# EdoardoBotta/RQ-VAE-Recommender

Hardware: AMD Instinct MI355X
Metric: item-embeddings quantized/sec (RQ-VAE fwd+bwd) (higher is better)
Workload: dtype f32 (MLP GEMMs f16x2-emulated)

## Files before the change

rq-vae-recommender_amd/csrc/wgrad_split.hip:

```cpp
#include "rqhip_common.h"

namespace rqhip {

typedef float ws_f32x16 __attribute__((ext_vector_type(16)));
typedef float ws_f32x4 __attribute__((ext_vector_type(4)));
typedef float ws_f32x2 __attribute__((ext_vector_type(2)));
typedef __bf16 ws_bf16x8 __attribute__((ext_vector_type(8)));
typedef __bf16 ws_bf16x2 __attribute__((ext_vector_type(2)));
typedef unsigned ws_u32x2 __attribute__((ext_vector_type(2)));

constexpr int kWsRows = 16;

#ifndef WS_PROBE
#define WS_PROBE 0
#endif

struct WgradSplitParams {
    const float *g, *y, *x;
    float *gm, *out;
    long long M;
    int N, K;
    int nslab_n, nslab_k, msplit;
    long long n_chunks;
    const unsigned *g_max, *x_max;
};

__device__ __forceinline__ void ws_split2(float a, float b, unsigned &h, unsigned &m, unsigned &l) {
    const ws_bf16x2 hh = __builtin_convertvector(ws_f32x2{a, b}, ws_bf16x2);
    h = __builtin_bit_cast(unsigned, hh);
    const float ra = a - __builtin_bit_cast(float, h << 16), rb = b - __builtin_bit_cast(float, h & 0xffff0000u);
    const ws_bf16x2 mm = __builtin_convertvector(ws_f32x2{ra, rb}, ws_bf16x2);
    m = __builtin_bit_cast(unsigned, mm);
    const float sa = ra - __builtin_bit_cast(float, m << 16), sb = rb - __builtin_bit_cast(float, m & 0xffff0000u);
    const ws_bf16x2 ll = __builtin_convertvector(ws_f32x2{sa, sb}, ws_bf16x2);
    l = __builtin_bit_cast(unsigned, ll);
}

typedef _Float16 ws_f16x8 __attribute__((ext_vector_type(8)));
typedef _Float16 ws_f16x2 __attribute__((ext_vector_type(2)));
__device__ __forceinline__ void ws_split2_f16(float a, float b, unsigned &h, unsigned &m) {
    const ws_f16x2 hh = __builtin_convertvector(ws_f32x2{a, b}, ws_f16x2);
    h = __builtin_bit_cast(unsigned, hh);
    const ws_f32x2 hf = __builtin_convertvector(hh, ws_f32x2);
    const ws_f16x2 mm = __builtin_convertvector(ws_f32x2{a - hf.x, b - hf.y}, ws_f16x2);
    m = __builtin_bit_cast(unsigned, mm);
}
__device__ __forceinline__ int ws_exp_of_bits(unsigned b) {
    b &= 0x7fffffffu;
    const int e = (int)(b >> 23);
    return (b == 0u || e == 255) ? 0 : (e == 0 ? -126 : e - 127) - 14;
}

__device__ __forceinline__ ws_f32x4 ws_load4(const float *p) {
    ws_f32x4 v;
    asm volatile("global_load_dwordx4 %0, %1, off" : "=v"(v) : "v"(p));
    return v;
}
template <int N>
__device__ __forceinline__ void ws_await(ws_f32x4 (&r)[4]) {
    asm volatile("s_waitcnt vmcnt(%4)" : "+v"(r[0]), "+v"(r[1]), "+v"(r[2]), "+v"(r[3]) : "n"(N) : "memory");
}

template <int TA, int TB, int WA, int WB, bool MASK, int NP>
__device__ __forceinline__ void wgrad_split_body(const WgradSplitParams &p, const int block) {
    constexpr int Nt = 32 * TA * WA, Kt = 32 * TB * WB, NT = 64 * WA * WB;
    constexpr int UNITS = Nt + Kt;
    constexpr int UQ = (UNITS + NT - 1) / NT;
    constexpr int SG = Nt / 4 + 4, SX = Kt / 4 + 4;
    constexpr int PART_G = NP * 2 * 4 * SG * 4, PART_X = NP * 2 * 4 * SX * 4;
    extern __shared__ __attribute__((aligned(16))) char ws_smem[];
    unsigned *sbuf = reinterpret_cast<unsigned *>(ws_smem);

    const int tid = threadIdx.x, lane = tid & 63, wave = tid >> 6;
    const int il = lane & 31, h = lane >> 5;
    const int wa = wave / WB, wb = wave % WB;
    const int nslabs = p.nslab_n * p.nslab_k;
    int slab, split;
    if ((p.msplit & 7) == 0) {
        const int xcd = block & 7, j = block >> 3;
        slab = j % nslabs;
        split = (j / nslabs) * 8 + xcd;
    } else {
        slab = block % nslabs;
        split = block / nslabs;
    }
    const int slab_n = slab / p.nslab_k, slab_k = slab % p.nslab_k;
    const int n0 = slab_n * Nt, k0 = slab_k * Kt;
    const long long r_begin = (p.n_chunks * split / p.msplit) * 32;
    long long r_end = (p.n_chunks * (split + 1) / p.msplit) * 32;
    if (r_end > p.M) r_end = p.M;
    const long long n_stage = (r_end - r_begin + kWsRows - 1) / kWsRows;
    const bool write_back = MASK && p.gm != nullptr && slab_k == 0;

    ws_f32x16 acc[TA][TB];
#pragma unroll
    for (int t = 0; t < TA; ++t)
#pragma unroll
        for (int u = 0; u < TB; ++u)
#pragma unroll
            for (int r = 0; r < 16; ++r) acc[t][u][r] = 0.0f;

    ws_f32x4 rv0[UQ][4], rv1[UQ][4], ry[MASK ? UQ : 1][4];
    int ue[NP == 2 ? UQ : 1][4];
#pragma unroll
    for (int q = 0; q < (NP == 2 ? UQ : 0); ++q) {
        const int u = tid + q * NT;
        const bool isg = u < Nt;
        const int idx = isg ? u : u - Nt, W = isg ? Nt : Kt;
        const int cq = idx % (W / 4);
        const unsigned *mxp = isg ? p.g_max : p.x_max;
        const int c0 = isg ? n0 : k0;
#pragma unroll
        for (int cc = 0; cc < 4; ++cc)
            ue[q][cc] = (mxp && ((UNITS % NT == 0) || u < UNITS)) ? ws_exp_of_bits(mxp[c0 + 4 * cq + cc]) : 0;
    }
    const long long n_full = (r_end - r_begin) / kWsRows;
    const float *cur[UQ][4];
    const float *ycur[MASK ? UQ : 1][4];
    size_t step16[UQ];
#pragma unroll
    for (int q = 0; q < UQ; ++q) {
        const int u = tid + q * NT;
        const bool live = (UNITS % NT == 0) || u < UNITS;
        const bool isg = u < Nt;
        const int idx = live ? (isg ? u : u - Nt) : 0, W = isg ? Nt : Kt;
        const int cq = idx % (W / 4), rq = idx / (W / 4);
        const int ld = isg ? p.N : p.K, c0 = isg ? n0 : k0;
        step16[q] = (size_t)kWsRows * ld;
#pragma unroll
        for (int j = 0; j < 4; ++j) {
            const size_t off = (size_t)(r_begin + 4 * rq + j) * ld + c0 + 4 * cq;
            cur[q][j] = (isg ? p.g : p.x) + off;
            if (MASK) ycur[q][j] = p.y + (isg ? off : (size_t)0);
        }
    }
    auto fetch_tail = [&](long long stage, ws_f32x4 (&rv)[UQ][4]) {
        const long long row0 = r_begin + stage * kWsRows;
#pragma unroll
        for (int q = 0; q < UQ; ++q) {
            const int u = tid + q * NT;
            const bool live = (UNITS % NT == 0) || u < UNITS;
            const bool isg = u < Nt;
            const int idx = live ? (isg ? u : u - Nt) : 0, W = isg ? Nt : Kt;
            const int cq = idx % (W / 4), rq = idx / (W / 4);
            const float *base = isg ? p.g : p.x;
            const int ld = isg ? p.N : p.K, c0 = isg ? n0 : k0;
#pragma unroll
            for (int j = 0; j < 4; ++j) {
                const long long row = row0 + 4 * rq + j;
                const bool ok = live && row < r_end;
                const size_t off = (size_t)(ok ? row : 0) * ld + c0 + 4 * cq;
                rv[q][j] = ok ? *reinterpret_cast<const ws_f32x4 *>(base + off) : ws_f32x4{0.f, 0.f, 0.f, 0.f};
                if (MASK) ry[q][j] = (ok && isg) ? *reinterpret_cast<const ws_f32x4 *>(p.y + off) : ws_f32x4{1.f, 1.f, 1.f, 1.f};
            }
        }
    };
    auto fetch = [&](long long stage, ws_f32x4 (&rv)[UQ][4]) {
        if (stage >= n_full) {
            fetch_tail(stage, rv);
            return;
        }
#pragma unroll
        for (int q = 0; q < UQ; ++q) {
            const int u = tid + q * NT;
            const bool live = (UNITS % NT == 0) || u < UNITS;
            const bool isg = u < Nt;
#pragma unroll
            for (int j = 0; j < 4; ++j) {
                if constexpr ((WS_PROBE & 2) != 0) {
                    rv[q][j] = ws_f32x4{1.f + (float)stage, 2.f, 3.f, 4.f};
                    if (MASK) ry[q][j] = ws_f32x4{1.f, 1.f, 1.f, 1.f};
                } else {
                    const ws_f32x4 v = *reinterpret_cast<const ws_f32x4 *>(cur[q][j]);
                    rv[q][j] = live ? v : ws_f32x4{0.f, 0.f, 0.f, 0.f};
                    if (MASK) {
                        const ws_f32x4 yv = *reinterpret_cast<const ws_f32x4 *>(ycur[q][j]);
                        ry[q][j] = (live && isg) ? yv : ws_f32x4{1.f, 1.f, 1.f, 1.f};
                    }
                }
                cur[q][j] += step16[q];
                if (MASK && isg) ycur[q][j] += step16[q];
            }
        }
    };
    auto stash = [&](long long stage, int buf, ws_f32x4 (&rv)[UQ][4]) {
        const long long row0 = r_begin + stage * kWsRows;
        unsigned *dst = sbuf + buf * (PART_G + PART_X);
        if (WS_PROBE & 1) return;
#pragma unroll
        for (int q = 0; q < UQ; ++q) {
            const int u = tid + q * NT;
            if (UNITS % NT != 0 && u >= UNITS) continue;
            const bool isg = u < Nt;
            const int idx = isg ? u : u - Nt, W = isg ? Nt : Kt;
            const int cq = idx % (W / 4), rq = idx / (W / 4);
            if (MASK && isg) {
#pragma unroll
                for (int j = 0; j < 4; ++j) {
                    rv[q][j].x = ry[q][j].x <= 0.0f ? 0.0f : rv[q][j].x;
                    rv[q][j].y = ry[q][j].y <= 0.0f ? 0.0f : rv[q][j].y;
                    rv[q][j].z = ry[q][j].z <= 0.0f ? 0.0f : rv[q][j].z;
                    rv[q][j].w = ry[q][j].w <= 0.0f ? 0.0f : rv[q][j].w;
                }
                if (write_back) {
#pragma unroll
                    for (int j = 0; j < 4; ++j) {
                        const long long row = row0 + 4 * rq + j;
                        if (row < r_end) *reinterpret_cast<ws_f32x4 *>(p.gm + (size_t)row * p.N + n0 + 4 * cq) = rv[q][j];
                    }
                }
            }
            unsigned *part = dst + (isg ? 0 : PART_G);
            const int oct = rq >> 1, half = rq & 1, S4 = 4 * (isg ? SG : SX);
#pragma unroll
            for (int cc = 0; cc < 4; ++cc) {
                unsigned h01, m01, l01 = 0u, h23, m23, l23 = 0u;
                if constexpr (NP == 2) {
                    ws_split2_f16(ldexpf(rv[q][0][cc], -ue[q][cc]), ldexpf(rv[q][1][cc], -ue[q][cc]), h01, m01);
                    ws_split2_f16(ldexpf(rv[q][2][cc], -ue[q][cc]), ldexpf(rv[q][3][cc], -ue[q][cc]), h23, m23);
                } else {
                    ws_split2(rv[q][0][cc], rv[q][1][cc], h01, m01, l01);
                    ws_split2(rv[q][2][cc], rv[q][3][cc], h23, m23, l23);
                }
                const int pos = cc * (S4 / 4) + cq;
                *reinterpret_cast<ws_u32x2 *>(part + ((0 * 2 + oct) * S4 + pos) * 4 + 2 * half) = ws_u32x2{h01, h23};
                *reinterpret_cast<ws_u32x2 *>(part + ((1 * 2 + oct) * S4 + pos) * 4 + 2 * half) = ws_u32x2{m01, m23};
                if (NP == 3) *reinterpret_cast<ws_u32x2 *>(part + ((2 * 2 + oct) * S4 + pos) * 4 + 2 * half) = ws_u32x2{l01, l23};
            }
        }
    };

    const bool stage_first = wave < (WA * WB) / 2;
    auto multiply = [&](int buf) {
        const ws_bf16x8 *gA = reinterpret_cast<const ws_bf16x8 *>(sbuf + buf * (PART_G + PART_X));
        const ws_bf16x8 *xB = reinterpret_cast<const ws_bf16x8 *>(sbuf + buf * (PART_G + PART_X) + PART_G);
        ws_bf16x8 a[TA][NP], b[TB][NP];
#pragma unroll
        for (int t = 0; t < TA; ++t)
#pragma unroll
            for (int pc = 0; pc < NP; ++pc)
                a[t][pc] = (WS_PROBE & 8) ? ws_bf16x8{(__bf16)(float)(t + buf), 1, 2, 3, 4, 5, 6, 7}
                                          : gA[(pc * 2 + h) * (4 * SG) + (il & 3) * SG + ((wa * 32 * TA + 32 * t + il) >> 2)];
#pragma unroll
        for (int u = 0; u < TB; ++u)
#pragma unroll
            for (int pc = 0; pc < NP; ++pc)
                b[u][pc] = (WS_PROBE & 8) ? ws_bf16x8{(__bf16)(float)(u + buf), 1, 2, 3, 4, 5, 6, 7}
                                          : xB[(pc * 2 + h) * (4 * SX) + (il & 3) * SX + ((wb * 32 * TB + 32 * u + il) >> 2)];
#pragma unroll
        for (int t = 0; t < TA; ++t)
#pragma unroll
            for (int u = 0; u < TB; ++u) {
                ws_f32x16 c16 = acc[t][u];
                if constexpr ((WS_PROBE & 4) != 0) {
                    c16[0] += (float)a[t][0][0] + (float)b[u][0][1] + (float)a[t][NP - 1][2] + (float)b[u][NP - 1][3];
                } else if constexpr (NP == 2) {
                    c16 = __builtin_amdgcn_mfma_f32_32x32x16_f16(__builtin_bit_cast(ws_f16x8, a[t][1]), __builtin_bit_cast(ws_f16x8, b[u][0]), c16, 0, 0, 0);
                    c16 = __builtin_amdgcn_mfma_f32_32x32x16_f16(__builtin_bit_cast(ws_f16x8, a[t][0]), __builtin_bit_cast(ws_f16x8, b[u][1]), c16, 0, 0, 0);
                    c16 = __builtin_amdgcn_mfma_f32_32x32x16_f16(__builtin_bit_cast(ws_f16x8, a[t][0]), __builtin_bit_cast(ws_f16x8, b[u][0]), c16, 0, 0, 0);
                } else {
                    c16 = __builtin_amdgcn_mfma_f32_32x32x16_bf16(a[t][1], b[u][1], c16, 0, 0, 0);
                    c16 = __builtin_amdgcn_mfma_f32_32x32x16_bf16(a[t][NP - 1], b[u][0], c16, 0, 0, 0);
                    c16 = __builtin_amdgcn_mfma_f32_32x32x16_bf16(a[t][0], b[u][NP - 1], c16, 0, 0, 0);
                    c16 = __builtin_amdgcn_mfma_f32_32x32x16_bf16(a[t][1], b[u][0], c16, 0, 0, 0);
                    c16 = __builtin_amdgcn_mfma_f32_32x32x16_bf16(a[t][0], b[u][1], c16, 0, 0, 0);
                    c16 = __builtin_amdgcn_mfma_f32_32x32x16_bf16(a[t][0], b[u][0], c16, 0, 0, 0);
                }
                acc[t][u] = c16;
            }
    };
    constexpr bool kTwoSets = !MASK && UQ == 1 && WS_PROBE == 0;
    if constexpr (!kTwoSets) {
        if (n_stage > 0) {
            fetch(0, rv0);
            stash(0, 0, rv0);
            if (n_stage > 1) fetch(1, rv0);
        }
        __syncthreads();
        for (long long c = 0; c < n_stage; ++c) {
            const int buf = (int)(c & 1);
            if (stage_first) {
                if (c + 1 < n_stage) stash(c + 1, buf ^ 1, rv0);
                if (c + 2 < n_stage) fetch(c + 2, rv0);
            }
            multiply(buf);
            if (!stage_first) {
                if (c + 1 < n_stage) stash(c + 1, buf ^ 1, rv0);
                if (c + 2 < n_stage) fetch(c + 2, rv0);
            }
            if (!(WS_PROBE & 16)) __syncthreads();
        }
    } else {
        auto load_set = [&](ws_f32x4 (&r)[UQ][4]) {
#pragma unroll
            for (int j = 0; j < 4; ++j) {
                r[0][j] = ws_load4(cur[0][j]);
                cur[0][j] += step16[0];
            }
        };
        long long c = 0;
        if (n_full >= 5) {
            load_set(rv0);
            load_set(rv1);
            ws_await<4>(rv0[0]);
            stash(0, 0, rv0);
            load_set(rv0);
            __syncthreads();
            if (stage_first) {
                for (; c + 4 < n_full; c += 2) {
                    ws_await<4>(rv1[0]);
                    stash(c + 1, 1, rv1);
                    load_set(rv1);
                    multiply(0);
                    __syncthreads();
                    ws_await<4>(rv0[0]);
                    stash(c + 2, 0, rv0);
                    load_set(rv0);
                    multiply(1);
                    __syncthreads();
                }
                ws_await<0>(rv1[0]);
                ws_await<0>(rv0[0]);
            } else {
                for (; c + 4 < n_full; c += 2) {
                    multiply(0);
                    ws_await<4>(rv1[0]);
                    stash(c + 1, 1, rv1);
                    load_set(rv1);
                    __syncthreads();
                    multiply(1);
                    ws_await<4>(rv0[0]);
                    stash(c + 2, 0, rv0);
                    load_set(rv0);
                    __syncthreads();
                }
                ws_await<0>(rv1[0]);
                ws_await<0>(rv0[0]);
            }
        } else {
            if (n_stage > 0) fetch(0, rv0);
            if (n_stage > 1) fetch(1, rv1);
            if (n_stage > 0) stash(0, 0, rv0);
            if (n_stage > 2) fetch(2, rv0);
            __syncthreads();
        }
        for (; c < n_stage; c += 2) {
            if (stage_first) {
                if (c + 1 < n_stage) stash(c + 1, 1, rv1);
                if (c + 3 < n_stage) fetch(c + 3, rv1);
            }
            multiply(0);
            if (!stage_first) {
                if (c + 1 < n_stage) stash(c + 1, 1, rv1);
                if (c + 3 < n_stage) fetch(c + 3, rv1);
            }
            __syncthreads();
            if (c + 1 >= n_stage) break;
            if (stage_first) {
                if (c + 2 < n_stage) stash(c + 2, 0, rv0);
                if (c + 4 < n_stage) fetch(c + 4, rv0);
            }
            multiply(1);
            if (!stage_first) {
                if (c + 2 < n_stage) stash(c + 2, 0, rv0);
                if (c + 4 < n_stage) fetch(c + 4, rv0);
            }
            __syncthreads();
        }
    }

    float *dst = p.out + (size_t)split * p.N * p.K;
    int ek[TB];
#pragma unroll
    for (int u = 0; u < TB; ++u) ek[u] = (NP == 2 && p.x_max) ? ws_exp_of_bits(p.x_max[k0 + wb * 32 * TB + 32 * u + il]) : 0;
    typedef unsigned ws_u32x4 __attribute__((ext_vector_type(4)));
    ws_u32x4 gb[TA][4];
#pragma unroll
    for (int t = 0; t < TA; ++t)
#pragma unroll
        for (int g4 = 0; g4 < 4; ++g4)
            gb[t][g4] = (NP == 2 && p.g_max) ? *reinterpret_cast<const ws_u32x4 *>(p.g_max + n0 + wa * 32 * TA + 32 * t + 8 * g4 + 4 * h)
                                             : ws_u32x4{0u, 0u, 0u, 0u};
#pragma unroll
    for (int t = 0; t < TA; ++t) {
#pragma unroll
        for (int u = 0; u < TB; ++u)
#pragma unroll
            for (int r = 0; r < 16; ++r) {
                const int n = n0 + wa * 32 * TA + 32 * t + 8 * (r >> 2) + 4 * h + (r & 3);
                const int k = k0 + wb * 32 * TB + 32 * u + il;
                float v = acc[t][u][r];
                if constexpr (NP == 2) v = ldexpf(v, ws_exp_of_bits(gb[t][r >> 2][r & 3]) + ek[u]);
                dst[(size_t)n * p.K + k] = v;
            }
    }
}

template <int TA, int TB, int WA, int WB, bool MASK, int NP>
__global__ __launch_bounds__(64 * WA * WB) void wgrad_split_kernel(const WgradSplitParams p) {
    wgrad_split_body<TA, TB, WA, WB, MASK, NP>(p, (int)blockIdx.x);
}

constexpr int kWsMaxJobs = 4;
struct WgradSplitJobs {
    WgradSplitParams p[kWsMaxJobs];
    int first[kWsMaxJobs];
    int n;
};
template <int TA, int TB, int WA, int WB, int NP>
__global__ __launch_bounds__(64 * WA * WB) void wgrad_split_jobs_kernel(const WgradSplitJobs jobs) {
    WgradSplitParams p = jobs.p[0];
    int first = 0;
#pragma unroll
    for (int j = 1; j < kWsMaxJobs; ++j)
        if (j < jobs.n && (int)blockIdx.x >= jobs.first[j]) {
            p = jobs.p[j];
            first = jobs.first[j];
        }
    wgrad_split_body<TA, TB, WA, WB, false, NP>(p, (int)blockIdx.x - first);
}

struct WgradSplitJobsMixed {
    WgradSplitJobs jobs;
    int cfg[kWsMaxJobs];
};
template <int NP>
__global__ __launch_bounds__(512) void wgrad_split_jobs_mixed_kernel(const WgradSplitJobsMixed m) {
    WgradSplitParams p = m.jobs.p[0];
    int first = 0, cfg = m.cfg[0];
#pragma unroll
    for (int j = 1; j < kWsMaxJobs; ++j)
        if (j < m.jobs.n && (int)blockIdx.x >= m.jobs.first[j]) {
            p = m.jobs.p[j];
            first = m.jobs.first[j];
            cfg = m.cfg[j];
        }
    if (cfg == 1) wgrad_split_body<2, 2, 2, 4, false, NP>(p, (int)blockIdx.x - first);
    else wgrad_split_body<2, 2, 4, 2, false, NP>(p, (int)blockIdx.x - first);
}

int wgrad_split_cfg(int N, int K) {
    if (N % 256 == 0 && K % 256 == 0) return 0;
    if (N % 128 == 0 && K % 256 == 0) return 1;
    if (N % 256 == 0 && K % 128 == 0) return 2;
    return -1;
}

template <int TA, int TB, int WA, int WB, int NP>
static int wgrad_split_go(const WgradSplitParams &p, bool mask, hipStream_t s) {
    constexpr int Nt = 32 * TA * WA, Kt = 32 * TB * WB;
    const size_t lds = (size_t)2 * (4 * (Nt / 4 + 4) + 4 * (Kt / 4 + 4)) * NP * 2 * 16;
    auto go = [&](auto kern) -> int {
        static LdsGrant grant;
        RQ_RETURN_IF_HIP(grant.ensure(reinterpret_cast<const void *>(kern), 160 * 1024));
        hipLaunchKernelGGL(kern, dim3(p.nslab_n * p.nslab_k * p.msplit), dim3(64 * WA * WB), lds, s, p);
        RQ_CHECK_LAUNCH("wgrad_split_kernel");
        return 0;
    };
    return mask ? go(wgrad_split_kernel<TA, TB, WA, WB, true, NP>) : go(wgrad_split_kernel<TA, TB, WA, WB, false, NP>);
}

int launch_wgrad_split(int cfg, const float *g, const float *y, const float *x, long long M, int N, int K, float *gm, float *out,
                       int nslab_n, int nslab_k, int msplit, const unsigned *g_max, const unsigned *x_max, hipStream_t s) {
    WgradSplitParams p;
    p.g = g; p.y = y; p.x = x; p.gm = gm; p.out = out;
    p.M = M; p.N = N; p.K = K; p.nslab_n = nslab_n; p.nslab_k = nslab_k; p.msplit = msplit;
    p.n_chunks = (M + 31) / 32;
    p.g_max = g_max;
    p.x_max = x_max;
    const bool mask = y != nullptr;
    if (g_max && x_max) {
        switch (cfg) {
            case 0: return wgrad_split_go<4, 2, 2, 4, 2>(p, mask, s);
            case 1: return wgrad_split_go<2, 2, 2, 4, 2>(p, mask, s);
            default: return wgrad_split_go<2, 2, 4, 2, 2>(p, mask, s);
        }
    }
    switch (cfg) {
        case 0: return wgrad_split_go<4, 2, 2, 4, 3>(p, mask, s);
        case 1: return wgrad_split_go<2, 2, 2, 4, 3>(p, mask, s);
        default: return wgrad_split_go<2, 2, 4, 2, 3>(p, mask, s);
    }
}

int launch_wgrad_split_jobs(int n, const float *const *g, const float *const *x, long long M, const int *N, const int *K, float *const *out,
                            int msplit, const unsigned *const *g_max, const unsigned *const *x_max, int half, hipStream_t s) {
    WgradSplitJobsMixed m;
    WgradSplitJobs &jobs = m.jobs;
    jobs.n = n;
    int blocks = 0;
    for (int j = 0; j < kWsMaxJobs; ++j) {
        const int i = j < n ? j : 0;
        const int cfg = half ? wgrad_split_cfg(N[i], K[i]) : 0;
        const int Nt = cfg == 1 ? 128 : 256, Kt = cfg == 2 ? 128 : 256;
        WgradSplitParams &p = jobs.p[j];
        p.g = g[i]; p.y = nullptr; p.x = x[i]; p.gm = nullptr; p.out = out[i];
        p.M = M; p.N = N[i]; p.K = K[i]; p.nslab_n = N[i] / Nt; p.nslab_k = K[i] / Kt; p.msplit = msplit;
        p.n_chunks = (M + 31) / 32;
        p.g_max = g_max[i]; p.x_max = x_max[i];
        m.cfg[j] = cfg;
        jobs.first[j] = blocks;
        if (j < n) blocks += p.nslab_n * p.nslab_k * msplit;
    }
    constexpr int NP = 2;
    static LdsGrant grant, grant_half;
    if (half) {
        constexpr int Nt = 128, Kt = 256;
        const size_t lds = (size_t)2 * (4 * (Nt / 4 + 4) + 4 * (Kt / 4 + 4)) * NP * 2 * 16;
        auto kern = wgrad_split_jobs_mixed_kernel<NP>;
        RQ_RETURN_IF_HIP(grant_half.ensure(reinterpret_cast<const void *>(kern), 160 * 1024));
        hipLaunchKernelGGL(kern, dim3(blocks), dim3(512), lds, s, m);
        RQ_CHECK_LAUNCH("wgrad_split_jobs_mixed_kernel");
        return 0;
    }
    constexpr int TA = 4, TB = 2, WA = 2, WB = 4, Nt = 32 * TA * WA, Kt = 32 * TB * WB;
    const size_t lds = (size_t)2 * (4 * (Nt / 4 + 4) + 4 * (Kt / 4 + 4)) * NP * 2 * 16;
    auto kern = wgrad_split_jobs_kernel<TA, TB, WA, WB, NP>;
    RQ_RETURN_IF_HIP(grant.ensure(reinterpret_cast<const void *>(kern), 160 * 1024));
    hipLaunchKernelGGL(kern, dim3(blocks), dim3(64 * WA * WB), lds, s, jobs);
    RQ_CHECK_LAUNCH("wgrad_split_jobs_kernel");
    return 0;
}

}
```

Measured before the change: 41.11 million.

## Deepen weight-gradient split-GEMM LDS pipeline to four slots per barrier

```diff
diff --git a/rq-vae-recommender_amd/csrc/wgrad_split.hip b/rq-vae-recommender_amd/csrc/wgrad_split.hip
--- a/rq-vae-recommender_amd/csrc/wgrad_split.hip
+++ b/rq-vae-recommender_amd/csrc/wgrad_split.hip
@@ -14,6 +14,11 @@
 #ifndef WS_PROBE
 #define WS_PROBE 0
 #endif
+constexpr int kWsProductDepth = WS_PROBE ? kWsRows : 2 * kWsRows;
+constexpr int ws_depth(bool mask, int np) { return (!mask && np == 2) ? kWsProductDepth : kWsRows; }
+constexpr size_t ws_lds_bytes(int Nt, int Kt, int np, int depth) {
+    return (size_t)2 * (depth / kWsRows) * (4 * (Nt / 4 + 4) + 4 * (Kt / 4 + 4)) * np * 2 * 16;
+}
 
 struct WgradSplitParams {
     const float *g, *y, *x;
@@ -61,7 +66,7 @@
     asm volatile("s_waitcnt vmcnt(%4)" : "+v"(r[0]), "+v"(r[1]), "+v"(r[2]), "+v"(r[3]) : "n"(N) : "memory");
 }
 
-template <int TA, int TB, int WA, int WB, bool MASK, int NP>
+template <int TA, int TB, int WA, int WB, bool MASK, int NP, int DEPTH>
 __device__ __forceinline__ void wgrad_split_body(const WgradSplitParams &p, const int block) {
     constexpr int Nt = 32 * TA * WA, Kt = 32 * TB * WB, NT = 64 * WA * WB;
     constexpr int UNITS = Nt + Kt;
@@ -70,6 +75,8 @@
     constexpr int PART_G = NP * 2 * 4 * SG * 4, PART_X = NP * 2 * 4 * SX * 4;
     extern __shared__ __attribute__((aligned(16))) char ws_smem[];
     unsigned *sbuf = reinterpret_cast<unsigned *>(ws_smem);
+    static_assert(DEPTH == kWsRows || (DEPTH == 2 * kWsRows && !MASK && NP == 2 && UQ == 1 && WS_PROBE == 0),
+                  "32-row intervals: the product path only");
 
     const int tid = threadIdx.x, lane = tid & 63, wave = tid >> 6;
     const int il = lane & 31, h = lane >> 5;
@@ -183,9 +190,20 @@
             }
         }
     };
-    auto stash = [&](long long stage, int buf, ws_f32x4 (&rv)[UQ][4]) {
+    constexpr unsigned kSlotBytes = 4u * (PART_G + PART_X);
+    unsigned woff[UQ][2];
+#pragma unroll
+    for (int q = 0; q < UQ; ++q) {
+        const int u = tid + q * NT;
+        const bool isg = u < Nt;
+        const int idx = isg ? u : u - Nt, W = isg ? Nt : Kt;
+        const int cq = idx % (W / 4), rq = idx / (W / 4);
+        woff[q][0] = 4u * (unsigned)((isg ? 0 : PART_G) + ((rq >> 1) * 4 * (isg ? SG : SX) + cq) * 4 + 2 * (rq & 1));
+        woff[q][1] = woff[q][0] + 2 * kSlotBytes;
+        asm volatile("" : "+v"(woff[q][1]));
+    }
+    auto stash = [&](long long stage, int slot, ws_f32x4 (&rv)[UQ][4]) {
         const long long row0 = r_begin + stage * kWsRows;
-        unsigned *dst = sbuf + buf * (PART_G + PART_X);
         if (WS_PROBE & 1) return;
 #pragma unroll
         for (int q = 0; q < UQ; ++q) {
@@ -210,8 +228,8 @@
                     }
                 }
             }
-            unsigned *part = dst + (isg ? 0 : PART_G);
-            const int oct = rq >> 1, half = rq & 1, S4 = 4 * (isg ? SG : SX);
+            const int S4 = 4 * (isg ? SG : SX);
+            unsigned *part = reinterpret_cast<unsigned *>(ws_smem + woff[q][slot >> 1] + (slot & 1) * kSlotBytes);
 #pragma unroll
             for (int cc = 0; cc < 4; ++cc) {
                 unsigned h01, m01, l01 = 0u, h23, m23, l23 = 0u;
@@ -222,31 +240,37 @@
                     ws_split2(rv[q][0][cc], rv[q][1][cc], h01, m01, l01);
                     ws_split2(rv[q][2][cc], rv[q][3][cc], h23, m23, l23);
                 }
-                const int pos = cc * (S4 / 4) + cq;
-                *reinterpret_cast<ws_u32x2 *>(part + ((0 * 2 + oct) * S4 + pos) * 4 + 2 * half) = ws_u32x2{h01, h23};
-                *reinterpret_cast<ws_u32x2 *>(part + ((1 * 2 + oct) * S4 + pos) * 4 + 2 * half) = ws_u32x2{m01, m23};
-                if (NP == 3) *reinterpret_cast<ws_u32x2 *>(part + ((2 * 2 + oct) * S4 + pos) * 4 + 2 * half) = ws_u32x2{l01, l23};
+                const int pos = cc * (S4 / 4);
+                *reinterpret_cast<ws_u32x2 *>(part + (0 * 2 * S4 + pos) * 4) = ws_u32x2{h01, h23};
+                *reinterpret_cast<ws_u32x2 *>(part + (1 * 2 * S4 + pos) * 4) = ws_u32x2{m01, m23};
+                if (NP == 3) *reinterpret_cast<ws_u32x2 *>(part + (2 * 2 * S4 + pos) * 4) = ws_u32x2{l01, l23};
             }
         }
     };
 
     const bool stage_first = wave < (WA * WB) / 2;
+    unsigned aoff[2], boff[2];
+    aoff[0] = 16u * (unsigned)(h * (4 * SG) + (il & 3) * SG + ((wa * 32 * TA + il) >> 2));
+    boff[0] = 16u * (unsigned)(h * (4 * SX) + (il & 3) * SX + ((wb * 32 * TB + il) >> 2)) + 4u * PART_G;
+    aoff[1] = aoff[0] + 2 * kSlotBytes;
+    boff[1] = boff[0] + 2 * kSlotBytes;
+    asm volatile("" : "+v"(aoff[1]), "+v"(boff[1]));
     auto multiply = [&](int buf) {
-        const ws_bf16x8 *gA = reinterpret_cast<const ws_bf16x8 *>(sbuf + buf * (PART_G + PART_X));
-        const ws_bf16x8 *xB = reinterpret_cast<const ws_bf16x8 *>(sbuf + buf * (PART_G + PART_X) + PART_G);
+        const ws_bf16x8 *gA = reinterpret_cast<const ws_bf16x8 *>(ws_smem + aoff[buf >> 1] + (buf & 1) * kSlotBytes);
+        const ws_bf16x8 *xB = reinterpret_cast<const ws_bf16x8 *>(ws_smem + boff[buf >> 1] + (buf & 1) * kSlotBytes);
         ws_bf16x8 a[TA][NP], b[TB][NP];
 #pragma unroll
         for (int t = 0; t < TA; ++t)
 #pragma unroll
             for (int pc = 0; pc < NP; ++pc)
                 a[t][pc] = (WS_PROBE & 8) ? ws_bf16x8{(__bf16)(float)(t + buf), 1, 2, 3, 4, 5, 6, 7}
-                                          : gA[(pc * 2 + h) * (4 * SG) + (il & 3) * SG + ((wa * 32 * TA + 32 * t + il) >> 2)];
+                                          : gA[pc * 2 * (4 * SG) + 8 * t];
 #pragma unroll
         for (int u = 0; u < TB; ++u)
 #pragma unroll
             for (int pc = 0; pc < NP; ++pc)
                 b[u][pc] = (WS_PROBE & 8) ? ws_bf16x8{(__bf16)(float)(u + buf), 1, 2, 3, 4, 5, 6, 7}
-                                          : xB[(pc * 2 + h) * (4 * SX) + (il & 3) * SX + ((wb * 32 * TB + 32 * u + il) >> 2)];
+                                          : xB[pc * 2 * (4 * SX) + 8 * u];
 #pragma unroll
         for (int t = 0; t < TA; ++t)
 #pragma unroll
@@ -268,9 +292,9 @@
                 }
                 acc[t][u] = c16;
             }
+        if constexpr (DEPTH != kWsRows) __builtin_amdgcn_sched_barrier(0);
     };
-    constexpr bool kTwoSets = !MASK && UQ == 1 && WS_PROBE == 0;
-    if constexpr (!kTwoSets) {
+    if constexpr (DEPTH == kWsRows) {
         if (n_stage > 0) {
             fetch(0, rv0);
             stash(0, 0, rv0);
@@ -298,72 +322,72 @@
                 cur[0][j] += step16[0];
             }
         };
+        auto refill = [&](int slot, ws_f32x4 (&r)[UQ][4]) {
+            ws_await<4>(r[0]);
+            stash(0, slot, r);
+            load_set(r);
+            __builtin_amdgcn_sched_barrier(0);
+        };
         long long c = 0;
-        if (n_full >= 5) {
+        if (n_full >= 8) {
             load_set(rv0);
             load_set(rv1);
-            ws_await<4>(rv0[0]);
-            stash(0, 0, rv0);
-            load_set(rv0);
+            refill(0, rv0);
+            refill(1, rv1);
             __syncthreads();
             if (stage_first) {
-                for (; c + 4 < n_full; c += 2) {
-                    ws_await<4>(rv1[0]);
-                    stash(c + 1, 1, rv1);
-                    load_set(rv1);
+                for (; c + 7 < n_full; c += 4) {
+                    refill(2, rv0);
                     multiply(0);
-                    __syncthreads();
-                    ws_await<4>(rv0[0]);
-                    stash(c + 2, 0, rv0);
-                    load_set(rv0);
+                    refill(3, rv1);
                     multiply(1);
                     __syncthreads();
-                }
-                ws_await<0>(rv1[0]);
-                ws_await<0>(rv0[0]);
+                    refill(0, rv0);
+                    multiply(2);
+                    refill(1, rv1);
+                    multiply(3);
+                    __syncthreads();
+                }
             } else {
-                for (; c + 4 < n_full; c += 2) {
+                for (; c + 7 < n_full; c += 4) {
                     multiply(0);
-                    ws_await<4>(rv1[0]);
-                    stash(c + 1, 1, rv1);
-                    load_set(rv1);
+                    refill(2, rv0);
+                    multiply(1);
+                    refill(3, rv1);
                     __syncthreads();
-                    multiply(1);
-                    ws_await<4>(rv0[0]);
-                    stash(c + 2, 0, rv0);
-                    load_set(rv0);
+                    multiply(2);
+                    refill(0, rv0);
+                    multiply(3);
+                    refill(1, rv1);
                     __syncthreads();
                 }
-                ws_await<0>(rv1[0]);
-                ws_await<0>(rv0[0]);
-            }
+            }
+            ws_await<0>(rv0[0]);
+            ws_await<0>(rv1[0]);
         } else {
             if (n_stage > 0) fetch(0, rv0);
             if (n_stage > 1) fetch(1, rv1);
             if (n_stage > 0) stash(0, 0, rv0);
             if (n_stage > 2) fetch(2, rv0);
+            if (n_stage > 1) stash(1, 1, rv1);
+            if (n_stage > 3) fetch(3, rv1);
             __syncthreads();
         }
         for (; c < n_stage; c += 2) {
+            const int rs = (int)(c & 2), wsl = rs ^ 2;
             if (stage_first) {
-                if (c + 1 < n_stage) stash(c + 1, 1, rv1);
-                if (c + 3 < n_stage) fetch(c + 3, rv1);
-            }
-            multiply(0);
+                if (c + 2 < n_stage) stash(c + 2, wsl, rv0);
+                if (c + 4 < n_stage) fetch(c + 4, rv0);
+                if (c + 3 < n_stage) stash(c + 3, wsl + 1, rv1);
+                if (c + 5 < n_stage) fetch(c + 5, rv1);
+            }
+            multiply(rs);
+            if (c + 1 < n_stage) multiply(rs + 1);
             if (!stage_first) {
-                if (c + 1 < n_stage) stash(c + 1, 1, rv1);
-                if (c + 3 < n_stage) fetch(c + 3, rv1);
-            }
-            __syncthreads();
-            if (c + 1 >= n_stage) break;
-            if (stage_first) {
-                if (c + 2 < n_stage) stash(c + 2, 0, rv0);
+                if (c + 2 < n_stage) stash(c + 2, wsl, rv0);
                 if (c + 4 < n_stage) fetch(c + 4, rv0);
-            }
-            multiply(1);
-            if (!stage_first) {
-                if (c + 2 < n_stage) stash(c + 2, 0, rv0);
-                if (c + 4 < n_stage) fetch(c + 4, rv0);
+                if (c + 3 < n_stage) stash(c + 3, wsl + 1, rv1);
+                if (c + 5 < n_stage) fetch(c + 5, rv1);
             }
             __syncthreads();
         }
@@ -398,7 +422,7 @@
 
 template <int TA, int TB, int WA, int WB, bool MASK, int NP>
 __global__ __launch_bounds__(64 * WA * WB) void wgrad_split_kernel(const WgradSplitParams p) {
-    wgrad_split_body<TA, TB, WA, WB, MASK, NP>(p, (int)blockIdx.x);
+    wgrad_split_body<TA, TB, WA, WB, MASK, NP, ws_depth(MASK, NP)>(p, (int)blockIdx.x);
 }
 
 constexpr int kWsMaxJobs = 4;
@@ -417,7 +441,7 @@
             p = jobs.p[j];
             first = jobs.first[j];
         }
-    wgrad_split_body<TA, TB, WA, WB, false, NP>(p, (int)blockIdx.x - first);
+    wgrad_split_body<TA, TB, WA, WB, false, NP, ws_depth(false, NP)>(p, (int)blockIdx.x - first);
 }
 
 struct WgradSplitJobsMixed {
@@ -435,8 +459,8 @@
             first = m.jobs.first[j];
             cfg = m.cfg[j];
         }
-    if (cfg == 1) wgrad_split_body<2, 2, 2, 4, false, NP>(p, (int)blockIdx.x - first);
-    else wgrad_split_body<2, 2, 4, 2, false, NP>(p, (int)blockIdx.x - first);
+    if (cfg == 1) wgrad_split_body<2, 2, 2, 4, false, NP, ws_depth(false, NP)>(p, (int)blockIdx.x - first);
+    else wgrad_split_body<2, 2, 4, 2, false, NP, ws_depth(false, NP)>(p, (int)blockIdx.x - first);
 }
 
 int wgrad_split_cfg(int N, int K) {
@@ -449,7 +473,7 @@
 template <int TA, int TB, int WA, int WB, int NP>
 static int wgrad_split_go(const WgradSplitParams &p, bool mask, hipStream_t s) {
     constexpr int Nt = 32 * TA * WA, Kt = 32 * TB * WB;
-    const size_t lds = (size_t)2 * (4 * (Nt / 4 + 4) + 4 * (Kt / 4 + 4)) * NP * 2 * 16;
+    const size_t lds = ws_lds_bytes(Nt, Kt, NP, ws_depth(mask, NP));
     auto go = [&](auto kern) -> int {
         static LdsGrant grant;
         RQ_RETURN_IF_HIP(grant.ensure(reinterpret_cast<const void *>(kern), 160 * 1024));
@@ -506,7 +530,7 @@
     static LdsGrant grant, grant_half;
     if (half) {
         constexpr int Nt = 128, Kt = 256;
-        const size_t lds = (size_t)2 * (4 * (Nt / 4 + 4) + 4 * (Kt / 4 + 4)) * NP * 2 * 16;
+        const size_t lds = ws_lds_bytes(Nt, Kt, NP, ws_depth(false, NP));
         auto kern = wgrad_split_jobs_mixed_kernel<NP>;
         RQ_RETURN_IF_HIP(grant_half.ensure(reinterpret_cast<const void *>(kern), 160 * 1024));
         hipLaunchKernelGGL(kern, dim3(blocks), dim3(512), lds, s, m);
@@ -514,7 +538,7 @@
         return 0;
     }
     constexpr int TA = 4, TB = 2, WA = 2, WB = 4, Nt = 32 * TA * WA, Kt = 32 * TB * WB;
-    const size_t lds = (size_t)2 * (4 * (Nt / 4 + 4) + 4 * (Kt / 4 + 4)) * NP * 2 * 16;
+    const size_t lds = ws_lds_bytes(Nt, Kt, NP, ws_depth(false, NP));
     auto kern = wgrad_split_jobs_kernel<TA, TB, WA, WB, NP>;
     RQ_RETURN_IF_HIP(grant.ensure(reinterpret_cast<const void *>(kern), 160 * 1024));
     hipLaunchKernelGGL(kern, dim3(blocks), dim3(64 * WA * WB), lds, s, jobs);
```

Result: no change. 41.18 million, median of 3 (+0.2%).
